# Xiuyu-Li/q-diffusion

Measured on NVIDIA H100. Metric: images_per_sec, higher is better.
Workload: dtype int8 (W4/W8 codes x A8 codes, int32 accumulate; fp32 norms/softmax)

## Files before the change

q-diffusion_b200/csrc/attention.cuh:

```cuda
#pragma once
#include <cuda_runtime.h>
#include <stdint.h>
#include "../../include/qdiff_b200.h"
#include "quant_math.cuh"

namespace qd {

template <bool A_SIGNED, bool B_SIGNED>
__device__ __forceinline__ void mma_i8_16832(int (&c)[4], const uint32_t (&a)[4], const uint32_t (&b)[2]) {
  if constexpr (A_SIGNED && B_SIGNED) {
    asm volatile("mma.sync.aligned.m16n8k32.row.col.s32.s8.s8.s32 {%0,%1,%2,%3}, {%4,%5,%6,%7}, {%8,%9}, {%0,%1,%2,%3};"
                 : "+r"(c[0]), "+r"(c[1]), "+r"(c[2]), "+r"(c[3])
                 : "r"(a[0]), "r"(a[1]), "r"(a[2]), "r"(a[3]), "r"(b[0]), "r"(b[1]));
  } else if constexpr (A_SIGNED && !B_SIGNED) {
    asm volatile("mma.sync.aligned.m16n8k32.row.col.s32.s8.u8.s32 {%0,%1,%2,%3}, {%4,%5,%6,%7}, {%8,%9}, {%0,%1,%2,%3};"
                 : "+r"(c[0]), "+r"(c[1]), "+r"(c[2]), "+r"(c[3])
                 : "r"(a[0]), "r"(a[1]), "r"(a[2]), "r"(a[3]), "r"(b[0]), "r"(b[1]));
  } else if constexpr (!A_SIGNED && B_SIGNED) {
    asm volatile("mma.sync.aligned.m16n8k32.row.col.s32.u8.s8.s32 {%0,%1,%2,%3}, {%4,%5,%6,%7}, {%8,%9}, {%0,%1,%2,%3};"
                 : "+r"(c[0]), "+r"(c[1]), "+r"(c[2]), "+r"(c[3])
                 : "r"(a[0]), "r"(a[1]), "r"(a[2]), "r"(a[3]), "r"(b[0]), "r"(b[1]));
  } else {
    asm volatile("mma.sync.aligned.m16n8k32.row.col.s32.u8.u8.s32 {%0,%1,%2,%3}, {%4,%5,%6,%7}, {%8,%9}, {%0,%1,%2,%3};"
                 : "+r"(c[0]), "+r"(c[1]), "+r"(c[2]), "+r"(c[3])
// ... 66 lines not shown
  l.kp = att_kp(DQ);
  l.vp = ATT_BN + 16;
  l.k_bytes = ATT_BN * l.kp;
  l.v_bytes = (DV + 8) * l.vp;
  l.zrk_off = 2 * l.k_bytes + 2 * l.v_bytes;
  l.total = l.zrk_off + 2 * ATT_BN * 4;
  return l;
}

template <bool MAGIC>
__device__ __forceinline__ float att_i2f(int s) {
  if constexpr (MAGIC) return __int_as_float(s + 0x4B400000) - 12582912.0f;
  else return (float)s;
}

template <int DQ, int DV, bool QK_SIGNED, bool V_SIGNED, bool SM16, int MINB, bool F16 = false>
__global__ void __launch_bounds__(ATT_WARPS * 32, MINB)
qattention_kernel(const qd_attention_desc p) {
  constexpr int KP = att_kp(DQ);
  constexpr int VP = ATT_BN + 16;
  constexpr int NKC = DQ / 32;
  constexpr int NDT = DV / 8 + 1;
  constexpr int KB = ATT_BN * KP, VB = (DV + 8) * VP;
  constexpr int ZB = ATT_BN * 4;
  constexpr bool MAGIC = DV <= 64;
  constexpr int RB = F16 ? 2 * DV : DV;
  constexpr int WPR = RB / 8;
  static_assert(!F16 || DV <= 64, "fp16 Q / K operands: d <= 64 keeps |S| below 2^22");
  extern __shared__ __align__(16) uint8_t att_smem[];

// ... 44 lines not shown
    const uint8_t* q0 = qbase + (long long)r0 * p.ld_q;
    const uint8_t* q1 = qbase + (long long)r1 * p.ld_q;
#pragma unroll
    for (int kc = 0; kc < NKC; ++kc) {
      const int c0 = kc * 32 + 8 * t, c1 = c0 + 4;
      qf[kc][0] = c0 < RB ? *reinterpret_cast<const uint32_t*>(q0 + c0) : 0u;
      qf[kc][1] = c0 < RB ? *reinterpret_cast<const uint32_t*>(q1 + c0) : 0u;
      qf[kc][2] = c1 < RB ? *reinterpret_cast<const uint32_t*>(q0 + c1) : 0u;
      qf[kc][3] = c1 < RB ? *reinterpret_cast<const uint32_t*>(q1 + c1) : 0u;
    }
  }
  const float c = p.sim_scale * 1.4426950408889634f;
  const bool has_zq = !F16 && p.zq != 0;
  const bool ragged = (p.Tk % ATT_BN) != 0;

  int mi0 = INT_MIN, mi1 = INT_MIN;
  float l0 = 0.f, l1 = 0.f;
  float off0 = 0.f, off1 = 0.f;
  int olo[NDT][4], ohi[SM16 ? NDT : 1][4];
#pragma unroll
  for (int i = 0; i < NDT; ++i) { olo[i][0] = olo[i][1] = olo[i][2] = olo[i][3] = 0; }
#pragma unroll
  for (int i = 0; i < (SM16 ? NDT : 1); ++i) { ohi[i][0] = ohi[i][1] = ohi[i][2] = ohi[i][3] = 0; }
  const float pmax = (float)p.p_qmax;
  const QuantK oqk = make_quantk(p.oq);

  int buf = 0;
  for (int pass = 0; pass < 2; ++pass) {
    if (pass == 1) {
      l0 += __shfl_xor_sync(0xffffffffu, l0, 1);
      l0 += __shfl_xor_sync(0xffffffffu, l0, 2);
      l1 += __shfl_xor_sync(0xffffffffu, l1, 1);
      l1 += __shfl_xor_sync(0xffffffffu, l1, 2);
      off0 = -(float)mi0 * c + log2f(1.0f / (l0 * p.delta_w));
      off1 = -(float)mi1 * c + log2f(1.0f / (l1 * p.delta_w));
    }
    for (int tile = 0; tile < ntiles; ++tile, buf ^= 1) {
      const int j0 = tile * ATT_BN;
      cp_async_wait_all();
      __syncthreads();
      if (tile + 1 < ntiles) prefetch(tile + 1, pass, buf ^ 1);
      else if (pass == 0) prefetch(0, 1, buf ^ 1);
      const uint8_t* sK = att_smem + buf * KB;
      const uint8_t* sV = att_smem + 2 * KB + buf * VB;
      const int* sZrk = reinterpret_cast<const int*>(att_smem + 2 * KB + 2 * VB + buf * ZB);

      int sacc[8][4];
#pragma unroll
      for (int nt = 0; nt < 8; ++nt) {
        sacc[nt][0] = sacc[nt][1] = sacc[nt][2] = sacc[nt][3] = 0;
        [[maybe_unused]] float facc[4] = {0.f, 0.f, 0.f, 0.f};
#pragma unroll
        for (int kc = 0; kc < NKC; ++kc) {
          const uint2 kk = *reinterpret_cast<const uint2*>(sK + (8 * nt + g) * KP + kc * 32 + 8 * t);
          const uint32_t bf[2] = {kk.x, kk.y};
          if constexpr (F16) mma_f16_16816(facc, qf[kc], bf);
          else mma_i8_16832<QK_SIGNED, QK_SIGNED>(sacc[nt], qf[kc], bf);
        }
        if constexpr (F16) {
          sacc[nt][0] = __float2int_rn(facc[0]); sacc[nt][1] = __float2int_rn(facc[1]);
          sacc[nt][2] = __float2int_rn(facc[2]); sacc[nt][3] = __float2int_rn(facc[3]);
        }
      }
      if (has_zq) {
#pragma unroll
        for (int nt = 0; nt < 8; ++nt) {
          const int2 z = *reinterpret_cast<const int2*>(sZrk + 8 * nt + 2 * t);
          sacc[nt][0] -= z.x; sacc[nt][1] -= z.y; sacc[nt][2] -= z.x; sacc[nt][3] -= z.y;
        }
      }
      if (ragged && tile == ntiles - 1) {
#pragma unroll
        for (int nt = 0; nt < 8; ++nt) {
          const int j = j0 + 8 * nt + 2 * t;
          if (j >= p.Tk) { sacc[nt][0] = -(1 << 21); sacc[nt][2] = -(1 << 21); }
          if (j + 1 >= p.Tk) { sacc[nt][1] = -(1 << 21); sacc[nt][3] = -(1 << 21); }
        }
      }
      if (pass == 0) {
        int tm0 = sacc[0][0], tm1 = sacc[0][2];
#pragma unroll
        for (int nt = 0; nt < 8; ++nt) {
          tm0 = max(tm0, max(sacc[nt][0], sacc[nt][1]));
          tm1 = max(tm1, max(sacc[nt][2], sacc[nt][3]));
        }
        tm0 = max(tm0, __shfl_xor_sync(0xffffffffu, tm0, 1));
        tm0 = max(tm0, __shfl_xor_sync(0xffffffffu, tm0, 2));
        tm1 = max(tm1, __shfl_xor_sync(0xffffffffu, tm1, 1));
        tm1 = max(tm1, __shfl_xor_sync(0xffffffffu, tm1, 2));
        if (tm0 > mi0) { l0 *= (mi0 == INT_MIN) ? 0.f : ex2_approx((float)(mi0 - tm0) * c); mi0 = tm0; }
        if (tm1 > mi1) { l1 *= (mi1 == INT_MIN) ? 0.f : ex2_approx((float)(mi1 - tm1) * c); mi1 = tm1; }
        const float b0 = -(float)mi0 * c, b1 = -(float)mi1 * c;
        float a0 = 0.f, a1 = 0.f;
#pragma unroll
        for (int nt = 0; nt < 8; ++nt) {
          a0 += ex2_approx(fmaf(att_i2f<MAGIC>(sacc[nt][0]), c, b0)) + ex2_approx(fmaf(att_i2f<MAGIC>(sacc[nt][1]), c, b0));
          a1 += ex2_approx(fmaf(att_i2f<MAGIC>(sacc[nt][2]), c, b1)) + ex2_approx(fmaf(att_i2f<MAGIC>(sacc[nt][3]), c, b1));
        }
        l0 += a0;
        l1 += a1;
      } else {
#pragma unroll
        for (int kc = 0; kc < 2; ++kc) {
          uint32_t plo[4], phi[4];
#pragma unroll
          for (int half = 0; half < 2; ++half) {
            const int ntA = 4 * kc + 2 * half, ntB = ntA + 1;
            uint32_t cd[8];
            const int sv[8] = {sacc[ntA][0], sacc[ntA][1], sacc[ntB][0], sacc[ntB][1],
                               sacc[ntA][2], sacc[ntA][3], sacc[ntB][2], sacc[ntB][3]};
#pragma unroll
            for (int e = 0; e < 8; ++e) {
              const float pr = ex2_approx(fmaf(att_i2f<MAGIC>(sv[e]), c, e < 4 ? off0 : off1));
              cd[e] = __float_as_uint(fminf(pr, pmax) + 12582912.0f);
            }
            plo[2 * half] = __byte_perm(__byte_perm(cd[0], cd[1], 0x0040), __byte_perm(cd[2], cd[3], 0x0040), 0x5410);
            plo[2 * half + 1] = __byte_perm(__byte_perm(cd[4], cd[5], 0x0040), __byte_perm(cd[6], cd[7], 0x0040), 0x5410);
            if constexpr (SM16) {
              phi[2 * half] = __byte_perm(__byte_perm(cd[0], cd[1], 0x0051), __byte_perm(cd[2], cd[3], 0x0051), 0x5410);
              phi[2 * half + 1] = __byte_perm(__byte_perm(cd[4], cd[5], 0x0051), __byte_perm(cd[6], cd[7], 0x0051), 0x5410);
            }
          }
#pragma unroll
          for (int nd = 0; nd < NDT; ++nd) {
            const uint8_t* vr = sV + (8 * nd + g) * VP + 32 * kc + 4 * t;
            const uint32_t bf[2] = {*reinterpret_cast<const uint32_t*>(vr), *reinterpret_cast<const uint32_t*>(vr + 16)};
            if (nd == NDT - 1) {
              mma_i8_16832<false, false>(olo[nd], plo, bf);
// ... 237 lines not shown
```

q-diffusion_b200/csrc/attention_wg.cuh:

```cuda
#pragma once
#include "attention.cuh"
#include "ptx.cuh"

namespace qd {

__device__ __forceinline__ void wgmma_ra_s8s8_n64(uint32_t* d, const uint32_t (&a)[4], uint64_t db, uint32_t scale_d) {
  asm volatile(
      "{\n\t.reg .pred p;\n\t"
      "setp.ne.b32 p, %37, 0;\n\t"
      "wgmma.mma_async.sync.aligned.m64n64k32.s32.s8.s8 "
      "{%0, %1, %2, %3, %4, %5, %6, %7, %8, %9, %10, %11, %12, %13, %14, %15, %16, %17, %18, %19, %20, %21, %22, %23, %24, %25, %26, %27, %28, %29, %30, %31}, {%32, %33, %34, %35}, %36, p;\n\t}\n"
      : "+r"(d[0]), "+r"(d[1]), "+r"(d[2]), "+r"(d[3]), "+r"(d[4]), "+r"(d[5]), "+r"(d[6]), "+r"(d[7]), "+r"(d[8]), "+r"(d[9]), "+r"(d[10]), "+r"(d[11]), "+r"(d[12]), "+r"(d[13]), "+r"(d[14]), "+r"(d[15]), "+r"(d[16]), "+r"(d[17]), "+r"(d[18]), "+r"(d[19]), "+r"(d[20]), "+r"(d[21]), "+r"(d[22]), "+r"(d[23]), "+r"(d[24]), "+r"(d[25]), "+r"(d[26]), "+r"(d[27]), "+r"(d[28]), "+r"(d[29]), "+r"(d[30]), "+r"(d[31])
      : "r"(a[0]), "r"(a[1]), "r"(a[2]), "r"(a[3]), "l"(db), "r"(scale_d));
}
__device__ __forceinline__ void wgmma_ra_u8u8_n64(uint32_t* d, const uint32_t (&a)[4], uint64_t db, uint32_t scale_d) {
  asm volatile(
      "{\n\t.reg .pred p;\n\t"
      "setp.ne.b32 p, %37, 0;\n\t"
      "wgmma.mma_async.sync.aligned.m64n64k32.s32.u8.u8 "
      "{%0, %1, %2, %3, %4, %5, %6, %7, %8, %9, %10, %11, %12, %13, %14, %15, %16, %17, %18, %19, %20, %21, %22, %23, %24, %25, %26, %27, %28, %29, %30, %31}, {%32, %33, %34, %35}, %36, p;\n\t}\n"
      : "+r"(d[0]), "+r"(d[1]), "+r"(d[2]), "+r"(d[3]), "+r"(d[4]), "+r"(d[5]), "+r"(d[6]), "+r"(d[7]), "+r"(d[8]), "+r"(d[9]), "+r"(d[10]), "+r"(d[11]), "+r"(d[12]), "+r"(d[13]), "+r"(d[14]), "+r"(d[15]), "+r"(d[16]), "+r"(d[17]), "+r"(d[18]), "+r"(d[19]), "+r"(d[20]), "+r"(d[21]), "+r"(d[22]), "+r"(d[23]), "+r"(d[24]), "+r"(d[25]), "+r"(d[26]), "+r"(d[27]), "+r"(d[28]), "+r"(d[29]), "+r"(d[30]), "+r"(d[31])
      : "r"(a[0]), "r"(a[1]), "r"(a[2]), "r"(a[3]), "l"(db), "r"(scale_d));
}
__device__ __forceinline__ void wgmma_ra_f16_n64(float* d, const uint32_t (&a)[4], uint64_t db, uint32_t scale_d) {
// ... 111 lines not shown
      "wgmma.mma_async.sync.aligned.m64n112k32.s32.u8.u8 "
      "{%0, %1, %2, %3, %4, %5, %6, %7, %8, %9, %10, %11, %12, %13, %14, %15, %16, %17, %18, %19, %20, %21, %22, %23, %24, %25, %26, %27, %28, %29, %30, %31, %32, %33, %34, %35, %36, %37, %38, %39, %40, %41, %42, %43, %44, %45, %46, %47, %48, %49, %50, %51, %52, %53, %54, %55}, {%56, %57, %58, %59}, %60, p;\n\t}\n"
      : "+r"(d[0]), "+r"(d[1]), "+r"(d[2]), "+r"(d[3]), "+r"(d[4]), "+r"(d[5]), "+r"(d[6]), "+r"(d[7]), "+r"(d[8]), "+r"(d[9]), "+r"(d[10]), "+r"(d[11]), "+r"(d[12]), "+r"(d[13]), "+r"(d[14]), "+r"(d[15]), "+r"(d[16]), "+r"(d[17]), "+r"(d[18]), "+r"(d[19]), "+r"(d[20]), "+r"(d[21]), "+r"(d[22]), "+r"(d[23]), "+r"(d[24]), "+r"(d[25]), "+r"(d[26]), "+r"(d[27]), "+r"(d[28]), "+r"(d[29]), "+r"(d[30]), "+r"(d[31]), "+r"(d[32]), "+r"(d[33]), "+r"(d[34]), "+r"(d[35]), "+r"(d[36]), "+r"(d[37]), "+r"(d[38]), "+r"(d[39]), "+r"(d[40]), "+r"(d[41]), "+r"(d[42]), "+r"(d[43]), "+r"(d[44]), "+r"(d[45]), "+r"(d[46]), "+r"(d[47]), "+r"(d[48]), "+r"(d[49]), "+r"(d[50]), "+r"(d[51]), "+r"(d[52]), "+r"(d[53]), "+r"(d[54]), "+r"(d[55])
      : "r"(a[0]), "r"(a[1]), "r"(a[2]), "r"(a[3]), "l"(db), "r"(scale_d));
}
__device__ __forceinline__ void wgmma_ra_u8s8_n112(uint32_t* d, const uint32_t (&a)[4], uint64_t db, uint32_t scale_d) {
  asm volatile(
      "{\n\t.reg .pred p;\n\t"
      "setp.ne.b32 p, %61, 0;\n\t"
      "wgmma.mma_async.sync.aligned.m64n112k32.s32.u8.s8 "
      "{%0, %1, %2, %3, %4, %5, %6, %7, %8, %9, %10, %11, %12, %13, %14, %15, %16, %17, %18, %19, %20, %21, %22, %23, %24, %25, %26, %27, %28, %29, %30, %31, %32, %33, %34, %35, %36, %37, %38, %39, %40, %41, %42, %43, %44, %45, %46, %47, %48, %49, %50, %51, %52, %53, %54, %55}, {%56, %57, %58, %59}, %60, p;\n\t}\n"
      : "+r"(d[0]), "+r"(d[1]), "+r"(d[2]), "+r"(d[3]), "+r"(d[4]), "+r"(d[5]), "+r"(d[6]), "+r"(d[7]), "+r"(d[8]), "+r"(d[9]), "+r"(d[10]), "+r"(d[11]), "+r"(d[12]), "+r"(d[13]), "+r"(d[14]), "+r"(d[15]), "+r"(d[16]), "+r"(d[17]), "+r"(d[18]), "+r"(d[19]), "+r"(d[20]), "+r"(d[21]), "+r"(d[22]), "+r"(d[23]), "+r"(d[24]), "+r"(d[25]), "+r"(d[26]), "+r"(d[27]), "+r"(d[28]), "+r"(d[29]), "+r"(d[30]), "+r"(d[31]), "+r"(d[32]), "+r"(d[33]), "+r"(d[34]), "+r"(d[35]), "+r"(d[36]), "+r"(d[37]), "+r"(d[38]), "+r"(d[39]), "+r"(d[40]), "+r"(d[41]), "+r"(d[42]), "+r"(d[43]), "+r"(d[44]), "+r"(d[45]), "+r"(d[46]), "+r"(d[47]), "+r"(d[48]), "+r"(d[49]), "+r"(d[50]), "+r"(d[51]), "+r"(d[52]), "+r"(d[53]), "+r"(d[54]), "+r"(d[55])
      : "r"(a[0]), "r"(a[1]), "r"(a[2]), "r"(a[3]), "l"(db), "r"(scale_d));
}

constexpr int ATW_STAGES = 3;
constexpr int ATW_THREADS = ATT_WARPS * 32;
__host__ __device__ constexpr int atw_nv(int DV) {
  return DV + 8 <= 24 ? 24 : DV + 8 <= 32 ? 32 : DV + 8 <= 48 ? 48 : DV + 8 <= 64 ? 64 : DV + 8 <= 80 ? 80 : DV + 8 <= 96 ? 96 : 112;
}
struct AtwSmem {
  int k_bytes, v_bytes, z_off, bar_off, total;
};
__host__ __device__ inline AtwSmem atw_smem(int P, int NV) {
  AtwSmem l;
  l.k_bytes = (ATT_BN * P + 1023) / 1024 * 1024;
  l.v_bytes = (NV * ATT_BN + 1023) / 1024 * 1024;
  l.z_off = ATW_STAGES * (l.k_bytes + l.v_bytes);
  l.bar_off = l.z_off + ATW_STAGES * ATT_BN * 4;
  l.total = l.bar_off + 2 * ATW_STAGES * 8 + 1024;
  return l;
}
__device__ __forceinline__ uint64_t atw_desc(uint32_t addr, int row_bytes) {
  const uint64_t layout = row_bytes == 128 ? 1 : row_bytes == 64 ? 2 : 3;
  uint64_t d = (uint64_t)((addr & 0x3FFFF) >> 4);
  d |= (uint64_t)1 << 16;
  d |= (uint64_t)((8 * row_bytes) >> 4) << 32;
  d |= layout << 62;
  return d;
}

template <int N, bool VS>
__device__ __forceinline__ void atw_pv(uint32_t* d, const uint32_t (&a)[4], uint64_t db) {
  if constexpr (VS) {
    if constexpr (N == 24) wgmma_ra_u8s8_n24(d, a, db, 1u);
    else if constexpr (N == 32) wgmma_ra_u8s8_n32(d, a, db, 1u);
    else if constexpr (N == 48) wgmma_ra_u8s8_n48(d, a, db, 1u);
    else if constexpr (N == 64) wgmma_ra_u8s8_n64(d, a, db, 1u);
    else if constexpr (N == 80) wgmma_ra_u8s8_n80(d, a, db, 1u);
    else if constexpr (N == 96) wgmma_ra_u8s8_n96(d, a, db, 1u);
    else wgmma_ra_u8s8_n112(d, a, db, 1u);
  } else {
    if constexpr (N == 24) wgmma_ra_u8u8_n24(d, a, db, 1u);
    else if constexpr (N == 32) wgmma_ra_u8u8_n32(d, a, db, 1u);
    else if constexpr (N == 48) wgmma_ra_u8u8_n48(d, a, db, 1u);
    else if constexpr (N == 64) wgmma_ra_u8u8_n64(d, a, db, 1u);
    else if constexpr (N == 80) wgmma_ra_u8u8_n80(d, a, db, 1u);
    else if constexpr (N == 96) wgmma_ra_u8u8_n96(d, a, db, 1u);
    else wgmma_ra_u8u8_n112(d, a, db, 1u);
  }
}

template <int DQ, int DV, bool QK_SIGNED, bool V_SIGNED, bool SM16, bool F16>
__global__ void __launch_bounds__(ATW_THREADS, 1)
qattention_wg_kernel(const __grid_constant__ CUtensorMap tmK, const __grid_constant__ CUtensorMap tmV,
                     const qd_attention_desc p, int P) {
  constexpr int NV = atw_nv(DV);
  constexpr int NKC = DQ / 32;
  constexpr int NDT = DV / 8 + 1;
  constexpr bool MAGIC = DV <= 64;
  constexpr int RB = F16 ? 2 * DV : DV;
  static_assert(!F16 || DV <= 64, "fp16 Q / K operands: d <= 64 keeps |S| below 2^22");
  extern __shared__ uint8_t atw_raw[];
  uint8_t* smem = atw_raw + (((smem_u32(atw_raw) + 1023u) & ~1023u) - smem_u32(atw_raw));
  const AtwSmem lay = atw_smem(P, NV);
  uint64_t* full = reinterpret_cast<uint64_t*>(smem + lay.bar_off);
  uint64_t* empty = full + ATW_STAGES;

  const int warp = threadIdx.x >> 5, lane = threadIdx.x & 31;
  const int g = lane >> 2, t = lane & 3;
  const int bh = blockIdx.y;
  const int b = bh / p.heads, h = bh - b * p.heads;
  const int row0 = blockIdx.x * ATT_BM + warp * 16;
  const int ntiles = (p.Tk + ATT_BN - 1) / ATT_BN;
  const int nloads = 2 * ntiles;
  const bool has_zq = !F16 && p.zq != 0;
  const int* zrk_g = reinterpret_cast<const int*>(p.ws) + (long long)bh * (long long)att_ws_stride(p.Tk);

  for (int i = threadIdx.x; i < ATW_STAGES * (NV - DV) * ATT_BN; i += ATW_THREADS) {
    const int s = i / ((NV - DV) * ATT_BN), r = (i / ATT_BN) % (NV - DV) + DV, c = i % ATT_BN;
    smem[ATW_STAGES * lay.k_bytes + s * lay.v_bytes + r * ATT_BN + c] = r == DV ? 1 : 0;
  }
  if (threadIdx.x == 0) {
    tma_prefetch_desc(&tmK);
    tma_prefetch_desc(&tmV);
    for (int s = 0; s < ATW_STAGES; ++s) {
      mbar_init(&full[s], 1);
      mbar_init(&empty[s], ATT_WARPS);
    }
    fence_mbar_init();
  }
  fence_proxy_async();
  __syncthreads();

  auto issue = [&](int L) {
    const int s = L % ATW_STAGES, pass = L / ntiles, tile = L - pass * ntiles;
    const int j0 = tile * ATT_BN;
    const uint32_t bytes = (uint32_t)(ATT_BN * P) + (pass ? (uint32_t)(ATT_BN * DV) : 0u) + (has_zq ? ATT_BN * 4u : 0u);
    mbar_arrive_expect_tx(&full[s], bytes);
    tma_load_2d(smem + s * lay.k_bytes, &tmK, &full[s], h * P, b * p.Tk + j0);
    if (pass) tma_load_2d(smem + ATW_STAGES * lay.k_bytes + s * lay.v_bytes, &tmV, &full[s], j0, bh * DV);
    if (has_zq) bulk_load_1d(smem + lay.z_off + s * ATT_BN * 4, zrk_g + j0, ATT_BN * 4, &full[s]);
  };
// ... 5 lines not shown
    const uint8_t* qbase = reinterpret_cast<const uint8_t*>(p.q) + (long long)b * p.Tq * p.ld_q + p.q_off + h * p.head_stride_q;
    const int r0 = min(row0 + g, p.Tq - 1), r1 = min(row0 + g + 8, p.Tq - 1);
    const uint8_t* q0 = qbase + (long long)r0 * p.ld_q;
    const uint8_t* q1 = qbase + (long long)r1 * p.ld_q;
#pragma unroll
    for (int kc = 0; kc < NKC; ++kc) {
      const int c0 = kc * 32 + 4 * t, c1 = c0 + 16;
      qf[kc][0] = c0 < RB ? *reinterpret_cast<const uint32_t*>(q0 + c0) : 0u;
      qf[kc][1] = c0 < RB ? *reinterpret_cast<const uint32_t*>(q1 + c0) : 0u;
      qf[kc][2] = c1 < RB ? *reinterpret_cast<const uint32_t*>(q0 + c1) : 0u;
      qf[kc][3] = c1 < RB ? *reinterpret_cast<const uint32_t*>(q1 + c1) : 0u;
    }
  }
  const float c = p.sim_scale * 1.4426950408889634f;
  const bool ragged = (p.Tk % ATT_BN) != 0;
  int mi0 = INT_MIN, mi1 = INT_MIN;
  float l0 = 0.f, l1 = 0.f;
  float off0 = 0.f, off1 = 0.f;
  uint32_t olo[NV / 2], ohi[SM16 ? NV / 2 : 1];
#pragma unroll
  for (int i = 0; i < NV / 2; ++i) olo[i] = 0u;
#pragma unroll
  for (int i = 0; i < (SM16 ? NV / 2 : 1); ++i) ohi[i] = 0u;
  const float pmax = (float)p.p_qmax;
  const QuantK oqk = make_quantk(p.oq);

  for (int pass = 0; pass < 2; ++pass) {
    if (pass == 1) {
      l0 += __shfl_xor_sync(0xffffffffu, l0, 1);
      l0 += __shfl_xor_sync(0xffffffffu, l0, 2);
      l1 += __shfl_xor_sync(0xffffffffu, l1, 1);
      l1 += __shfl_xor_sync(0xffffffffu, l1, 2);
      off0 = -(float)mi0 * c + log2f(1.0f / (l0 * p.delta_w));
      off1 = -(float)mi1 * c + log2f(1.0f / (l1 * p.delta_w));
    }
    for (int tile = 0; tile < ntiles; ++tile) {
      const int L = pass * ntiles + tile, st = L % ATW_STAGES;
      const uint32_t ph = (uint32_t)(L / ATW_STAGES) & 1u;
      const int j0 = tile * ATT_BN;
      mbar_wait(&full[st], ph);
      const uint64_t dK = atw_desc(smem_u32(smem + st * lay.k_bytes), P);
      const int* sZrk = reinterpret_cast<const int*>(smem + lay.z_off + st * ATT_BN * 4);

      int sacc[8][4];
      {
        uint32_t si[32];
        float sf[F16 ? 32 : 1];
        wgmma_fence();
#pragma unroll
        for (int kc = 0; kc < NKC; ++kc) {
          if constexpr (F16) wgmma_ra_f16_n64(sf, qf[kc], dK + (uint64_t)(2 * kc), kc ? 1u : 0u);
          else if constexpr (QK_SIGNED) wgmma_ra_s8s8_n64(si, qf[kc], dK + (uint64_t)(2 * kc), kc ? 1u : 0u);
          else wgmma_ra_u8u8_n64(si, qf[kc], dK + (uint64_t)(2 * kc), kc ? 1u : 0u);
        }
        wgmma_commit();
        wgmma_wait<0>();
        if constexpr (F16) {
#pragma unroll
          for (int i = 0; i < 32; ++i) asm volatile("" : "+f"(sf[i])::"memory");
#pragma unroll
          for (int i = 0; i < 32; ++i) sacc[i >> 2][i & 3] = __float2int_rn(sf[i]);
        } else {
#pragma unroll
          for (int i = 0; i < 32; ++i) asm volatile("" : "+r"(si[i])::"memory");
#pragma unroll
          for (int i = 0; i < 32; ++i) sacc[i >> 2][i & 3] = (int)si[i];
        }
      }
      if (has_zq) {
#pragma unroll
        for (int nt = 0; nt < 8; ++nt) {
          const int2 z = *reinterpret_cast<const int2*>(sZrk + 8 * nt + 2 * t);
          sacc[nt][0] -= z.x; sacc[nt][1] -= z.y; sacc[nt][2] -= z.x; sacc[nt][3] -= z.y;
        }
      }
      if (ragged && tile == ntiles - 1) {
#pragma unroll
        for (int nt = 0; nt < 8; ++nt) {
          const int j = j0 + 8 * nt + 2 * t;
          if (j >= p.Tk) { sacc[nt][0] = -(1 << 21); sacc[nt][2] = -(1 << 21); }
          if (j + 1 >= p.Tk) { sacc[nt][1] = -(1 << 21); sacc[nt][3] = -(1 << 21); }
        }
      }
      if (pass == 0) {
        int tm0 = sacc[0][0], tm1 = sacc[0][2];
#pragma unroll
        for (int nt = 0; nt < 8; ++nt) {
          tm0 = max(tm0, max(sacc[nt][0], sacc[nt][1]));
          tm1 = max(tm1, max(sacc[nt][2], sacc[nt][3]));
        }
        tm0 = max(tm0, __shfl_xor_sync(0xffffffffu, tm0, 1));
        tm0 = max(tm0, __shfl_xor_sync(0xffffffffu, tm0, 2));
        tm1 = max(tm1, __shfl_xor_sync(0xffffffffu, tm1, 1));
        tm1 = max(tm1, __shfl_xor_sync(0xffffffffu, tm1, 2));
        if (tm0 > mi0) { l0 *= (mi0 == INT_MIN) ? 0.f : ex2_approx((float)(mi0 - tm0) * c); mi0 = tm0; }
        if (tm1 > mi1) { l1 *= (mi1 == INT_MIN) ? 0.f : ex2_approx((float)(mi1 - tm1) * c); mi1 = tm1; }
        const float b0 = -(float)mi0 * c, b1 = -(float)mi1 * c;
        float a0 = 0.f, a1 = 0.f;
#pragma unroll
        for (int nt = 0; nt < 8; ++nt) {
          a0 += ex2_approx(fmaf(att_i2f<MAGIC>(sacc[nt][0]), c, b0)) + ex2_approx(fmaf(att_i2f<MAGIC>(sacc[nt][1]), c, b0));
          a1 += ex2_approx(fmaf(att_i2f<MAGIC>(sacc[nt][2]), c, b1)) + ex2_approx(fmaf(att_i2f<MAGIC>(sacc[nt][3]), c, b1));
        }
        l0 += a0;
        l1 += a1;
      } else {
        const uint64_t dV = atw_desc(smem_u32(smem + ATW_STAGES * lay.k_bytes + st * lay.v_bytes), ATT_BN);
        uint32_t plo[2][4], phi[2][4];
#pragma unroll
        for (int kc = 0; kc < 2; ++kc) {
#pragma unroll
          for (int half = 0; half < 2; ++half) {
            const int ntA = 4 * kc + 2 * half, ntB = ntA + 1;
            uint32_t cd[8];
            const int sv[8] = {sacc[ntA][0], sacc[ntA][1], sacc[ntB][0], sacc[ntB][1],
                               sacc[ntA][2], sacc[ntA][3], sacc[ntB][2], sacc[ntB][3]};
#pragma unroll
            for (int e = 0; e < 8; ++e) {
              const float pr = ex2_approx(fmaf(att_i2f<MAGIC>(sv[e]), c, e < 4 ? off0 : off1));
              cd[e] = __float_as_uint(fminf(pr, pmax) + 12582912.0f);
            }
            plo[kc][2 * half] = __byte_perm(__byte_perm(cd[0], cd[1], 0x0040), __byte_perm(cd[2], cd[3], 0x0040), 0x5410);
            plo[kc][2 * half + 1] = __byte_perm(__byte_perm(cd[4], cd[5], 0x0040), __byte_perm(cd[6], cd[7], 0x0040), 0x5410);
            if constexpr (SM16) {
              phi[kc][2 * half] = __byte_perm(__byte_perm(cd[0], cd[1], 0x0051), __byte_perm(cd[2], cd[3], 0x0051), 0x5410);
              phi[kc][2 * half + 1] = __byte_perm(__byte_perm(cd[4], cd[5], 0x0051), __byte_perm(cd[6], cd[7], 0x0051), 0x5410);
            }
          }
        }
        wgmma_fence();
#pragma unroll
        for (int kc = 0; kc < 2; ++kc) {
          atw_pv<NV, V_SIGNED>(olo, plo[kc], dV + (uint64_t)(2 * kc));
          if constexpr (SM16) atw_pv<NV, V_SIGNED>(ohi, phi[kc], dV + (uint64_t)(2 * kc));
        }
        wgmma_commit();
        wgmma_wait<0>();
#pragma unroll
        for (int i = 0; i < NV / 2; ++i) asm volatile("" : "+r"(olo[i])::"memory");
#pragma unroll
        for (int i = 0; i < (SM16 ? NV / 2 : 1); ++i) asm volatile("" : "+r"(ohi[i])::"memory");
      }
      __syncwarp();
      if (lane == 0) mbar_arrive(&empty[st]);
      if (threadIdx.x == 0 && L + ATW_STAGES < nloads) {
        mbar_wait(&empty[st], ph);
        issue(L + ATW_STAGES);
      }
      __syncwarp();
    }
  }

  float rs0 = (float)(int)olo[4 * (NDT - 1)], rs1 = (float)(int)olo[4 * (NDT - 1) + 2];
  if constexpr (SM16) { rs0 += 256.0f * (float)(int)ohi[4 * (NDT - 1)]; rs1 += 256.0f * (float)(int)ohi[4 * (NDT - 1) + 2]; }
  rs0 = __shfl_sync(0xffffffffu, rs0, lane & ~3);
  rs1 = __shfl_sync(0xffffffffu, rs1, lane & ~3);
  const int r0 = row0 + g, r1 = row0 + g + 8;
  const float z0 = (float)p.zv * rs0, z1 = (float)p.zv * rs1;
#pragma unroll
  for (int nd = 0; nd < NDT - 1; ++nd) {
    const int col = h * DV + 8 * nd + 2 * t;
    float v0 = (float)(int)olo[4 * nd], v1 = (float)(int)olo[4 * nd + 1], v2 = (float)(int)olo[4 * nd + 2], v3 = (float)(int)olo[4 * nd + 3];
    if constexpr (SM16) {
      v0 += 256.0f * (float)(int)ohi[4 * nd]; v1 += 256.0f * (float)(int)ohi[4 * nd + 1];
      v2 += 256.0f * (float)(int)ohi[4 * nd + 2]; v3 += 256.0f * (float)(int)ohi[4 * nd + 3];
    }
// ... 20 lines not shown
```

q-diffusion_b200/csrc/engine.cu:

```cuda
#include <cuda.h>
#include <cuda_runtime.h>
#include <cudaTypedefs.h>

#include <atomic>
#include <cstdarg>
#include <cstdio>
#include <cstdlib>
#include <cstring>
#include <mutex>
#include <new>
#include <utility>
#include <vector>

#include "../../include/qdiff_b200.h"
#include "attention.cuh"
#include "attention_wg.cuh"
#include "elem.cuh"
#include "gemm_i8.cuh"

namespace {

thread_local char g_err[512] = "";
std::atomic<long long> g_launches{0};
constexpr int kMaxDevices = 64;
// ... 645 lines not shown
  static const int forced_mma = [] { const char* e = getenv("QDIFF_ATTENTION"); return (e && !strcmp(e, "mma")) ? 1 : 0; }();
  if (forced_mma) return false;
  const int P = d.head_stride_q, rb = d.qk_f16 ? 2 * d.d : d.d;
  if (d.d != 16 && d.d != 24 && d.d != 32 && d.d != 40 && d.d != 48 && d.d != 64 && d.d != 80 && d.d != 96) return false;
  if (d.qk_f16 && d.d > 64) return false;
  if (d.qk_f16 && d.d == 48) return false;
  if ((P != 32 && P != 64 && P != 128) || P < rb || d.head_stride_k != P) return false;
  if (d.q_off != 0 || d.k_off != 0 || (d.ld_k & 15) || (((uintptr_t)d.k) & 15) || (((uintptr_t)d.vt) & 15)) return false;
  if (d.v_off != 0 || d.head_stride_v != d.d || d.v_batch_stride != (long long)d.heads * d.d * d.ld_vt) return false;
  if (d.zq != 0 && !d.qk_f16 && !d.ws) return false;
  return true;
}

template <int DQ, int DV, bool QS, bool VS, bool S16, bool F16>
int launch_attention_wg_inst(const qd_attention_desc& d, cudaStream_t s) {
  auto kern = qd::qattention_wg_kernel<DQ, DV, QS, VS, S16, F16>;
  const int P = d.head_stride_q;
  const qd::AtwSmem lay = qd::atw_smem(P, qd::atw_nv(DV));
  static std::atomic<unsigned long long> optin{0};
  if (int rc = ensure_smem_optin(kern, 227 * 1024, optin, "attention_wg")) return rc;
  CUtensorMap tmK, tmV;
  {
    cuuint64_t dims[2] = {(cuuint64_t)d.ld_k, (cuuint64_t)d.B * d.Tk};
    cuuint64_t strides[1] = {(cuuint64_t)d.ld_k};
    cuuint32_t box[2] = {(cuuint32_t)P, (cuuint32_t)qd::ATT_BN};
    if (int rc = encode_u8_map(&tmK, d.k, 2, dims, strides, box, P)) return rc;
  }
  {
    cuuint64_t dims[2] = {(cuuint64_t)d.ld_vt, (cuuint64_t)d.B * d.heads * d.d};
    cuuint64_t strides[1] = {(cuuint64_t)d.ld_vt};
    cuuint32_t box[2] = {(cuuint32_t)qd::ATT_BN, (cuuint32_t)d.d};
// ... 332 lines not shown
```

Measured before the change: 3.710.

## Restructure wgmma attention loop with atomic stage release, fp32 scores, deeper pipeline

Rewrites the warpgroup attention main loop as a single flattened loop over load indices. Stage reuse is now signalled by a shared-memory atomic counter: the last warp to finish a stage issues the next TMA load, replacing the empty-mbarrier wait done by thread 0. PV accumulators start through the wgmma scale_d flag instead of explicit zeroing. The pipeline depth goes from three to four stages, and small-head instantiations get launch bounds that allow two blocks per SM. Fp16 score paths keep float scores instead of rounding to int, which removes the conversions but changes numerics slightly. The atomic release scheme adds a correctness risk, and the extra stage and higher occupancy target add smem and register pressure.

```diff
diff --git a/q-diffusion_b200/csrc/attention.cuh b/q-diffusion_b200/csrc/attention.cuh
--- a/q-diffusion_b200/csrc/attention.cuh
+++ b/q-diffusion_b200/csrc/attention.cuh
@@ -1,6 +1,7 @@
 #pragma once
 #include <cuda_runtime.h>
 #include <stdint.h>
+#include <type_traits>
 #include "../../include/qdiff_b200.h"
 #include "quant_math.cuh"
 
@@ -104,6 +105,17 @@
   else return (float)s;
 }
 
+template <bool F16>
+using att_score_t = std::conditional_t<F16, float, int>;
+template <bool MAGIC>
+__device__ __forceinline__ float att_s2f(int s) { return att_i2f<MAGIC>(s); }
+template <bool MAGIC>
+__device__ __forceinline__ float att_s2f(float s) { return s; }
+__device__ __forceinline__ int att_smax(int a, int b) { return max(a, b); }
+__device__ __forceinline__ float att_smax(float a, float b) { return fmaxf(a, b); }
+__device__ __forceinline__ int att_lowest(int) { return INT_MIN; }
+__device__ __forceinline__ float att_lowest(float) { return -INFINITY; }
+
 template <int DQ, int DV, bool QK_SIGNED, bool V_SIGNED, bool SM16, int MINB, bool F16 = false>
 __global__ void __launch_bounds__(ATT_WARPS * 32, MINB)
 qattention_kernel(const qd_attention_desc p) {
@@ -178,7 +190,8 @@
   const bool has_zq = !F16 && p.zq != 0;
   const bool ragged = (p.Tk % ATT_BN) != 0;
 
-  int mi0 = INT_MIN, mi1 = INT_MIN;
+  using SV = att_score_t<F16>;
+  SV mi0 = att_lowest(SV{}), mi1 = att_lowest(SV{});
   float l0 = 0.f, l1 = 0.f;
   float off0 = 0.f, off1 = 0.f;
   int olo[NDT][4], ohi[SM16 ? NDT : 1][4];
@@ -209,21 +222,16 @@
       const uint8_t* sV = att_smem + 2 * KB + buf * VB;
       const int* sZrk = reinterpret_cast<const int*>(att_smem + 2 * KB + 2 * VB + buf * ZB);
 
-      int sacc[8][4];
+      SV sacc[8][4];
 #pragma unroll
       for (int nt = 0; nt < 8; ++nt) {
         sacc[nt][0] = sacc[nt][1] = sacc[nt][2] = sacc[nt][3] = 0;
-        [[maybe_unused]] float facc[4] = {0.f, 0.f, 0.f, 0.f};
 #pragma unroll
         for (int kc = 0; kc < NKC; ++kc) {
           const uint2 kk = *reinterpret_cast<const uint2*>(sK + (8 * nt + g) * KP + kc * 32 + 8 * t);
           const uint32_t bf[2] = {kk.x, kk.y};
-          if constexpr (F16) mma_f16_16816(facc, qf[kc], bf);
+          if constexpr (F16) mma_f16_16816(sacc[nt], qf[kc], bf);
           else mma_i8_16832<QK_SIGNED, QK_SIGNED>(sacc[nt], qf[kc], bf);
-        }
-        if constexpr (F16) {
-          sacc[nt][0] = __float2int_rn(facc[0]); sacc[nt][1] = __float2int_rn(facc[1]);
-          sacc[nt][2] = __float2int_rn(facc[2]); sacc[nt][3] = __float2int_rn(facc[3]);
         }
       }
       if (has_zq) {
@@ -242,24 +250,24 @@
         }
       }
       if (pass == 0) {
-        int tm0 = sacc[0][0], tm1 = sacc[0][2];
+        SV tm0 = sacc[0][0], tm1 = sacc[0][2];
 #pragma unroll
         for (int nt = 0; nt < 8; ++nt) {
-          tm0 = max(tm0, max(sacc[nt][0], sacc[nt][1]));
-          tm1 = max(tm1, max(sacc[nt][2], sacc[nt][3]));
-        }
-        tm0 = max(tm0, __shfl_xor_sync(0xffffffffu, tm0, 1));
-        tm0 = max(tm0, __shfl_xor_sync(0xffffffffu, tm0, 2));
-        tm1 = max(tm1, __shfl_xor_sync(0xffffffffu, tm1, 1));
-        tm1 = max(tm1, __shfl_xor_sync(0xffffffffu, tm1, 2));
-        if (tm0 > mi0) { l0 *= (mi0 == INT_MIN) ? 0.f : ex2_approx((float)(mi0 - tm0) * c); mi0 = tm0; }
-        if (tm1 > mi1) { l1 *= (mi1 == INT_MIN) ? 0.f : ex2_approx((float)(mi1 - tm1) * c); mi1 = tm1; }
+          tm0 = att_smax(tm0, att_smax(sacc[nt][0], sacc[nt][1]));
+          tm1 = att_smax(tm1, att_smax(sacc[nt][2], sacc[nt][3]));
+        }
+        tm0 = att_smax(tm0, __shfl_xor_sync(0xffffffffu, tm0, 1));
+        tm0 = att_smax(tm0, __shfl_xor_sync(0xffffffffu, tm0, 2));
+        tm1 = att_smax(tm1, __shfl_xor_sync(0xffffffffu, tm1, 1));
+        tm1 = att_smax(tm1, __shfl_xor_sync(0xffffffffu, tm1, 2));
+        if (tm0 > mi0) { l0 *= (mi0 == att_lowest(SV{})) ? 0.f : ex2_approx((float)(mi0 - tm0) * c); mi0 = tm0; }
+        if (tm1 > mi1) { l1 *= (mi1 == att_lowest(SV{})) ? 0.f : ex2_approx((float)(mi1 - tm1) * c); mi1 = tm1; }
         const float b0 = -(float)mi0 * c, b1 = -(float)mi1 * c;
         float a0 = 0.f, a1 = 0.f;
 #pragma unroll
         for (int nt = 0; nt < 8; ++nt) {
-          a0 += ex2_approx(fmaf(att_i2f<MAGIC>(sacc[nt][0]), c, b0)) + ex2_approx(fmaf(att_i2f<MAGIC>(sacc[nt][1]), c, b0));
-          a1 += ex2_approx(fmaf(att_i2f<MAGIC>(sacc[nt][2]), c, b1)) + ex2_approx(fmaf(att_i2f<MAGIC>(sacc[nt][3]), c, b1));
+          a0 += ex2_approx(fmaf(att_s2f<MAGIC>(sacc[nt][0]), c, b0)) + ex2_approx(fmaf(att_s2f<MAGIC>(sacc[nt][1]), c, b0));
+          a1 += ex2_approx(fmaf(att_s2f<MAGIC>(sacc[nt][2]), c, b1)) + ex2_approx(fmaf(att_s2f<MAGIC>(sacc[nt][3]), c, b1));
         }
         l0 += a0;
         l1 += a1;
@@ -271,11 +279,11 @@
           for (int half = 0; half < 2; ++half) {
             const int ntA = 4 * kc + 2 * half, ntB = ntA + 1;
             uint32_t cd[8];
-            const int sv[8] = {sacc[ntA][0], sacc[ntA][1], sacc[ntB][0], sacc[ntB][1],
-                               sacc[ntA][2], sacc[ntA][3], sacc[ntB][2], sacc[ntB][3]};
+            const SV sv[8] = {sacc[ntA][0], sacc[ntA][1], sacc[ntB][0], sacc[ntB][1],
+                              sacc[ntA][2], sacc[ntA][3], sacc[ntB][2], sacc[ntB][3]};
 #pragma unroll
             for (int e = 0; e < 8; ++e) {
-              const float pr = ex2_approx(fmaf(att_i2f<MAGIC>(sv[e]), c, e < 4 ? off0 : off1));
+              const float pr = ex2_approx(fmaf(att_s2f<MAGIC>(sv[e]), c, e < 4 ? off0 : off1));
               cd[e] = __float_as_uint(fminf(pr, pmax) + 12582912.0f);
             }
             plo[2 * half] = __byte_perm(__byte_perm(cd[0], cd[1], 0x0040), __byte_perm(cd[2], cd[3], 0x0040), 0x5410);
diff --git a/q-diffusion_b200/csrc/attention_wg.cuh b/q-diffusion_b200/csrc/attention_wg.cuh
--- a/q-diffusion_b200/csrc/attention_wg.cuh
+++ b/q-diffusion_b200/csrc/attention_wg.cuh
@@ -149,7 +149,7 @@
       : "r"(a[0]), "r"(a[1]), "r"(a[2]), "r"(a[3]), "l"(db), "r"(scale_d));
 }
 
-constexpr int ATW_STAGES = 3;
+constexpr int ATW_STAGES = 4;
 constexpr int ATW_THREADS = ATT_WARPS * 32;
 __host__ __device__ constexpr int atw_nv(int DV) {
   return DV + 8 <= 24 ? 24 : DV + 8 <= 32 ? 32 : DV + 8 <= 48 ? 48 : DV + 8 <= 64 ? 64 : DV + 8 <= 80 ? 80 : DV + 8 <= 96 ? 96 : 112;
@@ -163,7 +163,7 @@
   l.v_bytes = (NV * ATT_BN + 1023) / 1024 * 1024;
   l.z_off = ATW_STAGES * (l.k_bytes + l.v_bytes);
   l.bar_off = l.z_off + ATW_STAGES * ATT_BN * 4;
-  l.total = l.bar_off + 2 * ATW_STAGES * 8 + 1024;
+  l.total = l.bar_off + ATW_STAGES * 8 + ATW_STAGES * 4 + 1024;
   return l;
 }
 __device__ __forceinline__ uint64_t atw_desc(uint32_t addr, int row_bytes) {
@@ -176,28 +176,28 @@
 }
 
 template <int N, bool VS>
-__device__ __forceinline__ void atw_pv(uint32_t* d, const uint32_t (&a)[4], uint64_t db) {
+__device__ __forceinline__ void atw_pv(uint32_t* d, const uint32_t (&a)[4], uint64_t db, uint32_t scale_d) {
   if constexpr (VS) {
-    if constexpr (N == 24) wgmma_ra_u8s8_n24(d, a, db, 1u);
-    else if constexpr (N == 32) wgmma_ra_u8s8_n32(d, a, db, 1u);
-    else if constexpr (N == 48) wgmma_ra_u8s8_n48(d, a, db, 1u);
-    else if constexpr (N == 64) wgmma_ra_u8s8_n64(d, a, db, 1u);
-    else if constexpr (N == 80) wgmma_ra_u8s8_n80(d, a, db, 1u);
-    else if constexpr (N == 96) wgmma_ra_u8s8_n96(d, a, db, 1u);
-    else wgmma_ra_u8s8_n112(d, a, db, 1u);
+    if constexpr (N == 24) wgmma_ra_u8s8_n24(d, a, db, scale_d);
+    else if constexpr (N == 32) wgmma_ra_u8s8_n32(d, a, db, scale_d);
+    else if constexpr (N == 48) wgmma_ra_u8s8_n48(d, a, db, scale_d);
+    else if constexpr (N == 64) wgmma_ra_u8s8_n64(d, a, db, scale_d);
+    else if constexpr (N == 80) wgmma_ra_u8s8_n80(d, a, db, scale_d);
+    else if constexpr (N == 96) wgmma_ra_u8s8_n96(d, a, db, scale_d);
+    else wgmma_ra_u8s8_n112(d, a, db, scale_d);
   } else {
-    if constexpr (N == 24) wgmma_ra_u8u8_n24(d, a, db, 1u);
-    else if constexpr (N == 32) wgmma_ra_u8u8_n32(d, a, db, 1u);
-    else if constexpr (N == 48) wgmma_ra_u8u8_n48(d, a, db, 1u);
-    else if constexpr (N == 64) wgmma_ra_u8u8_n64(d, a, db, 1u);
-    else if constexpr (N == 80) wgmma_ra_u8u8_n80(d, a, db, 1u);
-    else if constexpr (N == 96) wgmma_ra_u8u8_n96(d, a, db, 1u);
-    else wgmma_ra_u8u8_n112(d, a, db, 1u);
-  }
-}
-
-template <int DQ, int DV, bool QK_SIGNED, bool V_SIGNED, bool SM16, bool F16>
-__global__ void __launch_bounds__(ATW_THREADS, 1)
+    if constexpr (N == 24) wgmma_ra_u8u8_n24(d, a, db, scale_d);
+    else if constexpr (N == 32) wgmma_ra_u8u8_n32(d, a, db, scale_d);
+    else if constexpr (N == 48) wgmma_ra_u8u8_n48(d, a, db, scale_d);
+    else if constexpr (N == 64) wgmma_ra_u8u8_n64(d, a, db, scale_d);
+    else if constexpr (N == 80) wgmma_ra_u8u8_n80(d, a, db, scale_d);
+    else if constexpr (N == 96) wgmma_ra_u8u8_n96(d, a, db, scale_d);
+    else wgmma_ra_u8u8_n112(d, a, db, scale_d);
+  }
+}
+
+template <int DQ, int DV, bool QK_SIGNED, bool V_SIGNED, bool SM16, bool F16, int MINB>
+__global__ void __launch_bounds__(ATW_THREADS, MINB)
 qattention_wg_kernel(const __grid_constant__ CUtensorMap tmK, const __grid_constant__ CUtensorMap tmV,
                      const qd_attention_desc p, int P) {
   constexpr int NV = atw_nv(DV);
@@ -206,11 +206,12 @@
   constexpr bool MAGIC = DV <= 64;
   constexpr int RB = F16 ? 2 * DV : DV;
   static_assert(!F16 || DV <= 64, "fp16 Q / K operands: d <= 64 keeps |S| below 2^22");
+  using SV = att_score_t<F16>;
   extern __shared__ uint8_t atw_raw[];
   uint8_t* smem = atw_raw + (((smem_u32(atw_raw) + 1023u) & ~1023u) - smem_u32(atw_raw));
   const AtwSmem lay = atw_smem(P, NV);
   uint64_t* full = reinterpret_cast<uint64_t*>(smem + lay.bar_off);
-  uint64_t* empty = full + ATW_STAGES;
+  int* released = reinterpret_cast<int*>(full + ATW_STAGES);
 
   const int warp = threadIdx.x >> 5, lane = threadIdx.x & 31;
   const int g = lane >> 2, t = lane & 3;
@@ -231,7 +232,7 @@
     tma_prefetch_desc(&tmV);
     for (int s = 0; s < ATW_STAGES; ++s) {
       mbar_init(&full[s], 1);
-      mbar_init(&empty[s], ATT_WARPS);
+      released[s] = 0;
     }
     fence_mbar_init();
   }
@@ -267,19 +268,44 @@
   }
   const float c = p.sim_scale * 1.4426950408889634f;
   const bool ragged = (p.Tk % ATT_BN) != 0;
-  int mi0 = INT_MIN, mi1 = INT_MIN;
+  SV mi0 = att_lowest(SV{}), mi1 = att_lowest(SV{});
   float l0 = 0.f, l1 = 0.f;
   float off0 = 0.f, off1 = 0.f;
   uint32_t olo[NV / 2], ohi[SM16 ? NV / 2 : 1];
-#pragma unroll
-  for (int i = 0; i < NV / 2; ++i) olo[i] = 0u;
-#pragma unroll
-  for (int i = 0; i < (SM16 ? NV / 2 : 1); ++i) ohi[i] = 0u;
   const float pmax = (float)p.p_qmax;
   const QuantK oqk = make_quantk(p.oq);
 
-  for (int pass = 0; pass < 2; ++pass) {
-    if (pass == 1) {
+  auto issue_s = [&](SV (&s)[8][4], int L) {
+    const int st = L % ATW_STAGES;
+    mbar_wait(&full[st], (uint32_t)(L / ATW_STAGES) & 1u);
+    const uint64_t dK = atw_desc(smem_u32(smem + st * lay.k_bytes), P);
+    wgmma_fence();
+#pragma unroll
+    for (int kc = 0; kc < NKC; ++kc) {
+      if constexpr (F16) wgmma_ra_f16_n64(&s[0][0], qf[kc], dK + (uint64_t)(2 * kc), kc ? 1u : 0u);
+      else if constexpr (QK_SIGNED) wgmma_ra_s8s8_n64(reinterpret_cast<uint32_t*>(&s[0][0]), qf[kc], dK + (uint64_t)(2 * kc), kc ? 1u : 0u);
+      else wgmma_ra_u8u8_n64(reinterpret_cast<uint32_t*>(&s[0][0]), qf[kc], dK + (uint64_t)(2 * kc), kc ? 1u : 0u);
+    }
+    wgmma_commit();
+  };
+
+  auto release = [&](int R) {
+    __syncwarp();
+    if (lane == 0) {
+      const int s = R % ATW_STAGES;
+      __threadfence_block();
+      const int n = atomicAdd(&released[s], 1);
+      if (n == ATT_WARPS * (R / ATW_STAGES + 1) - 1 && R + ATW_STAGES < nloads) {
+        __threadfence_block();
+        issue(R + ATW_STAGES);
+      }
+    }
+  };
+
+  auto softmax_pv = [&](SV (&sacc)[8][4], int L) {
+    const int pass = L >= ntiles ? 1 : 0, tile = L - pass * ntiles, st = L % ATW_STAGES;
+    const int j0 = tile * ATT_BN;
+    if (L == ntiles) {
       l0 += __shfl_xor_sync(0xffffffffu, l0, 1);
       l0 += __shfl_xor_sync(0xffffffffu, l0, 2);
       l1 += __shfl_xor_sync(0xffffffffu, l1, 1);
@@ -287,122 +313,96 @@
       off0 = -(float)mi0 * c + log2f(1.0f / (l0 * p.delta_w));
       off1 = -(float)mi1 * c + log2f(1.0f / (l1 * p.delta_w));
     }
-    for (int tile = 0; tile < ntiles; ++tile) {
-      const int L = pass * ntiles + tile, st = L % ATW_STAGES;
-      const uint32_t ph = (uint32_t)(L / ATW_STAGES) & 1u;
-      const int j0 = tile * ATT_BN;
-      mbar_wait(&full[st], ph);
-      const uint64_t dK = atw_desc(smem_u32(smem + st * lay.k_bytes), P);
-      const int* sZrk = reinterpret_cast<const int*>(smem + lay.z_off + st * ATT_BN * 4);
-
-      int sacc[8][4];
-      {
-        uint32_t si[32];
-        float sf[F16 ? 32 : 1];
-        wgmma_fence();
-#pragma unroll
-        for (int kc = 0; kc < NKC; ++kc) {
-          if constexpr (F16) wgmma_ra_f16_n64(sf, qf[kc], dK + (uint64_t)(2 * kc), kc ? 1u : 0u);
-          else if constexpr (QK_SIGNED) wgmma_ra_s8s8_n64(si, qf[kc], dK + (uint64_t)(2 * kc), kc ? 1u : 0u);
-          else wgmma_ra_u8u8_n64(si, qf[kc], dK + (uint64_t)(2 * kc), kc ? 1u : 0u);
-        }
-        wgmma_commit();
-        wgmma_wait<0>();
-        if constexpr (F16) {
-#pragma unroll
-          for (int i = 0; i < 32; ++i) asm volatile("" : "+f"(sf[i])::"memory");
-#pragma unroll
-          for (int i = 0; i < 32; ++i) sacc[i >> 2][i & 3] = __float2int_rn(sf[i]);
-        } else {
-#pragma unroll
-          for (int i = 0; i < 32; ++i) asm volatile("" : "+r"(si[i])::"memory");
-#pragma unroll
-          for (int i = 0; i < 32; ++i) sacc[i >> 2][i & 3] = (int)si[i];
-        }
-      }
-      if (has_zq) {
-#pragma unroll
-        for (int nt = 0; nt < 8; ++nt) {
-          const int2 z = *reinterpret_cast<const int2*>(sZrk + 8 * nt + 2 * t);
-          sacc[nt][0] -= z.x; sacc[nt][1] -= z.y; sacc[nt][2] -= z.x; sacc[nt][3] -= z.y;
-        }
-      }
-      if (ragged && tile == ntiles - 1) {
-#pragma unroll
-        for (int nt = 0; nt < 8; ++nt) {
-          const int j = j0 + 8 * nt + 2 * t;
-          if (j >= p.Tk) { sacc[nt][0] = -(1 << 21); sacc[nt][2] = -(1 << 21); }
-          if (j + 1 >= p.Tk) { sacc[nt][1] = -(1 << 21); sacc[nt][3] = -(1 << 21); }
-        }
-      }
-      if (pass == 0) {
-        int tm0 = sacc[0][0], tm1 = sacc[0][2];
-#pragma unroll
-        for (int nt = 0; nt < 8; ++nt) {
-          tm0 = max(tm0, max(sacc[nt][0], sacc[nt][1]));
-          tm1 = max(tm1, max(sacc[nt][2], sacc[nt][3]));
-        }
-        tm0 = max(tm0, __shfl_xor_sync(0xffffffffu, tm0, 1));
-        tm0 = max(tm0, __shfl_xor_sync(0xffffffffu, tm0, 2));
-        tm1 = max(tm1, __shfl_xor_sync(0xffffffffu, tm1, 1));
-        tm1 = max(tm1, __shfl_xor_sync(0xffffffffu, tm1, 2));
-        if (tm0 > mi0) { l0 *= (mi0 == INT_MIN) ? 0.f : ex2_approx((float)(mi0 - tm0) * c); mi0 = tm0; }
-        if (tm1 > mi1) { l1 *= (mi1 == INT_MIN) ? 0.f : ex2_approx((float)(mi1 - tm1) * c); mi1 = tm1; }
-        const float b0 = -(float)mi0 * c, b1 = -(float)mi1 * c;
-        float a0 = 0.f, a1 = 0.f;
-#pragma unroll
-        for (int nt = 0; nt < 8; ++nt) {
-          a0 += ex2_approx(fmaf(att_i2f<MAGIC>(sacc[nt][0]), c, b0)) + ex2_approx(fmaf(att_i2f<MAGIC>(sacc[nt][1]), c, b0));
-          a1 += ex2_approx(fmaf(att_i2f<MAGIC>(sacc[nt][2]), c, b1)) + ex2_approx(fmaf(att_i2f<MAGIC>(sacc[nt][3]), c, b1));
-        }
-        l0 += a0;
-        l1 += a1;
-      } else {
-        const uint64_t dV = atw_desc(smem_u32(smem + ATW_STAGES * lay.k_bytes + st * lay.v_bytes), ATT_BN);
-        uint32_t plo[2][4], phi[2][4];
-#pragma unroll
-        for (int kc = 0; kc < 2; ++kc) {
-#pragma unroll
-          for (int half = 0; half < 2; ++half) {
-            const int ntA = 4 * kc + 2 * half, ntB = ntA + 1;
-            uint32_t cd[8];
-            const int sv[8] = {sacc[ntA][0], sacc[ntA][1], sacc[ntB][0], sacc[ntB][1],
-                               sacc[ntA][2], sacc[ntA][3], sacc[ntB][2], sacc[ntB][3]};
-#pragma unroll
-            for (int e = 0; e < 8; ++e) {
-              const float pr = ex2_approx(fmaf(att_i2f<MAGIC>(sv[e]), c, e < 4 ? off0 : off1));
-              cd[e] = __float_as_uint(fminf(pr, pmax) + 12582912.0f);
-            }
-            plo[kc][2 * half] = __byte_perm(__byte_perm(cd[0], cd[1], 0x0040), __byte_perm(cd[2], cd[3], 0x0040), 0x5410);
-            plo[kc][2 * half + 1] = __byte_perm(__byte_perm(cd[4], cd[5], 0x0040), __byte_perm(cd[6], cd[7], 0x0040), 0x5410);
-            if constexpr (SM16) {
-              phi[kc][2 * half] = __byte_perm(__byte_perm(cd[0], cd[1], 0x0051), __byte_perm(cd[2], cd[3], 0x0051), 0x5410);
-              phi[kc][2 * half + 1] = __byte_perm(__byte_perm(cd[4], cd[5], 0x0051), __byte_perm(cd[6], cd[7], 0x0051), 0x5410);
-            }
+    const int* sZrk = reinterpret_cast<const int*>(smem + lay.z_off + st * ATT_BN * 4);
+    if (has_zq) {
+#pragma unroll
+      for (int nt = 0; nt < 8; ++nt) {
+        const int2 z = *reinterpret_cast<const int2*>(sZrk + 8 * nt + 2 * t);
+        sacc[nt][0] -= z.x; sacc[nt][1] -= z.y; sacc[nt][2] -= z.x; sacc[nt][3] -= z.y;
+      }
+    }
+    if (ragged && tile == ntiles - 1) {
+#pragma unroll
+      for (int nt = 0; nt < 8; ++nt) {
+        const int j = j0 + 8 * nt + 2 * t;
+        if (j >= p.Tk) { sacc[nt][0] = -(1 << 21); sacc[nt][2] = -(1 << 21); }
+        if (j + 1 >= p.Tk) { sacc[nt][1] = -(1 << 21); sacc[nt][3] = -(1 << 21); }
+      }
+    }
+    if (pass == 0) {
+      SV tm0 = sacc[0][0], tm1 = sacc[0][2];
+#pragma unroll
+      for (int nt = 0; nt < 8; ++nt) {
+        tm0 = att_smax(tm0, att_smax(sacc[nt][0], sacc[nt][1]));
+        tm1 = att_smax(tm1, att_smax(sacc[nt][2], sacc[nt][3]));
+      }
+      tm0 = att_smax(tm0, __shfl_xor_sync(0xffffffffu, tm0, 1));
+      tm0 = att_smax(tm0, __shfl_xor_sync(0xffffffffu, tm0, 2));
+      tm1 = att_smax(tm1, __shfl_xor_sync(0xffffffffu, tm1, 1));
+      tm1 = att_smax(tm1, __shfl_xor_sync(0xffffffffu, tm1, 2));
+      if (tm0 > mi0) { l0 *= (mi0 == att_lowest(SV{})) ? 0.f : ex2_approx((float)(mi0 - tm0) * c); mi0 = tm0; }
+      if (tm1 > mi1) { l1 *= (mi1 == att_lowest(SV{})) ? 0.f : ex2_approx((float)(mi1 - tm1) * c); mi1 = tm1; }
+      const float b0 = -(float)mi0 * c, b1 = -(float)mi1 * c;
+      float a0 = 0.f, a1 = 0.f;
+#pragma unroll
+      for (int nt = 0; nt < 8; ++nt) {
+        a0 += ex2_approx(fmaf(att_s2f<MAGIC>(sacc[nt][0]), c, b0)) + ex2_approx(fmaf(att_s2f<MAGIC>(sacc[nt][1]), c, b0));
+        a1 += ex2_approx(fmaf(att_s2f<MAGIC>(sacc[nt][2]), c, b1)) + ex2_approx(fmaf(att_s2f<MAGIC>(sacc[nt][3]), c, b1));
+      }
+      l0 += a0;
+      l1 += a1;
+    } else {
+      const uint64_t dV = atw_desc(smem_u32(smem + ATW_STAGES * lay.k_bytes + st * lay.v_bytes), ATT_BN);
+      uint32_t plo[2][4], phi[2][4];
+#pragma unroll
+      for (int kc = 0; kc < 2; ++kc) {
+#pragma unroll
+        for (int half = 0; half < 2; ++half) {
+          const int ntA = 4 * kc + 2 * half, ntB = ntA + 1;
+          uint32_t cd[8];
+          const SV sv[8] = {sacc[ntA][0], sacc[ntA][1], sacc[ntB][0], sacc[ntB][1],
+                            sacc[ntA][2], sacc[ntA][3], sacc[ntB][2], sacc[ntB][3]};
+#pragma unroll
+          for (int e = 0; e < 8; ++e) {
+            const float pr = ex2_approx(fmaf(att_s2f<MAGIC>(sv[e]), c, e < 4 ? off0 : off1));
+            cd[e] = __float_as_uint(fminf(pr, pmax) + 12582912.0f);
+          }
+          plo[kc][2 * half] = __byte_perm(__byte_perm(cd[0], cd[1], 0x0040), __byte_perm(cd[2], cd[3], 0x0040), 0x5410);
+          plo[kc][2 * half + 1] = __byte_perm(__byte_perm(cd[4], cd[5], 0x0040), __byte_perm(cd[6], cd[7], 0x0040), 0x5410);
+          if constexpr (SM16) {
+            phi[kc][2 * half] = __byte_perm(__byte_perm(cd[0], cd[1], 0x0051), __byte_perm(cd[2], cd[3], 0x0051), 0x5410);
+            phi[kc][2 * half + 1] = __byte_perm(__byte_perm(cd[4], cd[5], 0x0051), __byte_perm(cd[6], cd[7], 0x0051), 0x5410);
           }
         }
-        wgmma_fence();
-#pragma unroll
-        for (int kc = 0; kc < 2; ++kc) {
-          atw_pv<NV, V_SIGNED>(olo, plo[kc], dV + (uint64_t)(2 * kc));
-          if constexpr (SM16) atw_pv<NV, V_SIGNED>(ohi, phi[kc], dV + (uint64_t)(2 * kc));
-        }
-        wgmma_commit();
-        wgmma_wait<0>();
-#pragma unroll
-        for (int i = 0; i < NV / 2; ++i) asm volatile("" : "+r"(olo[i])::"memory");
-#pragma unroll
-        for (int i = 0; i < (SM16 ? NV / 2 : 1); ++i) asm volatile("" : "+r"(ohi[i])::"memory");
-      }
-      __syncwarp();
-      if (lane == 0) mbar_arrive(&empty[st]);
-      if (threadIdx.x == 0 && L + ATW_STAGES < nloads) {
-        mbar_wait(&empty[st], ph);
-        issue(L + ATW_STAGES);
-      }
-      __syncwarp();
-    }
-  }
+      }
+      wgmma_fence();
+#pragma unroll
+      for (int kc = 0; kc < 2; ++kc) {
+        const uint32_t acc = (kc || L > ntiles) ? 1u : 0u;
+        atw_pv<NV, V_SIGNED>(olo, plo[kc], dV + (uint64_t)(2 * kc), acc);
+        if constexpr (SM16) atw_pv<NV, V_SIGNED>(ohi, phi[kc], dV + (uint64_t)(2 * kc), acc);
+      }
+      wgmma_commit();
+    }
+  };
+
+  for (int L = 0; L < nloads; ++L) {
+    SV sacc[8][4];
+    issue_s(sacc, L);
+    wgmma_wait<0>();
+#pragma unroll
+    for (int i = 0; i < 32; ++i) {
+      if constexpr (F16) asm volatile("" : "+f"(sacc[i >> 2][i & 3])::"memory");
+      else asm volatile("" : "+r"(sacc[i >> 2][i & 3])::"memory");
+    }
+    softmax_pv(sacc, L);
+    wgmma_wait<0>();
+    release(L);
+  }
+#pragma unroll
+  for (int i = 0; i < NV / 2; ++i) asm volatile("" : "+r"(olo[i])::"memory");
+#pragma unroll
+  for (int i = 0; i < (SM16 ? NV / 2 : 1); ++i) asm volatile("" : "+r"(ohi[i])::"memory");
 
   float rs0 = (float)(int)olo[4 * (NDT - 1)], rs1 = (float)(int)olo[4 * (NDT - 1) + 2];
   if constexpr (SM16) { rs0 += 256.0f * (float)(int)ohi[4 * (NDT - 1)]; rs1 += 256.0f * (float)(int)ohi[4 * (NDT - 1) + 2]; }
diff --git a/q-diffusion_b200/csrc/engine.cu b/q-diffusion_b200/csrc/engine.cu
--- a/q-diffusion_b200/csrc/engine.cu
+++ b/q-diffusion_b200/csrc/engine.cu
@@ -683,7 +683,8 @@
 
 template <int DQ, int DV, bool QS, bool VS, bool S16, bool F16>
 int launch_attention_wg_inst(const qd_attention_desc& d, cudaStream_t s) {
-  auto kern = qd::qattention_wg_kernel<DQ, DV, QS, VS, S16, F16>;
+  constexpr int MINB = DV <= 40 ? 2 : 1;
+  auto kern = qd::qattention_wg_kernel<DQ, DV, QS, VS, S16, F16, MINB>;
   const int P = d.head_stride_q;
   const qd::AtwSmem lay = qd::atw_smem(P, qd::atw_nv(DV));
   static std::atomic<unsigned long long> optin{0};
```

Result: faster. 4.096, median of 6 (+10.4%).
